# DongSky/few-shot-vit

Hardware: AMD Instinct MI355X
Metric: episodes_per_sec_5way_5shot_visformer_s (higher is better)
Workload: dtype bf16; 1 GPU; BASELINE configs[1]: Visformer-S (visformer_micro_80) miniImageNet-shaped 5-way 5-shot episodic eval, 15 query/class, 80x80 fp32 NCHW episodes resident in HBM, procedural weights + calibrated BN; images_per_episode=100, encoder_chunk_images=12800, distinct_episode_batches=16, parallelism=episode-parallel x1, one all-reduce of accuracy stats, ranks_seen=1, per_rank_eps=4521.1

## Files before the change

### few-shot-vit_amd/_lib.py

```python
import ctypes as C
import os

_HERE = os.path.dirname(os.path.abspath(__file__))
LIB_PATH = os.path.join(_HERE, 'libfsvit.so')

F32, BF16, F16, BF16X2, F16X2 = 0, 1, 2, 3, 4
ACT_NONE, ACT_GELU, ACT_LRELU = 0, 1, 2
HEAD_COS, HEAD_SQR, HEAD_DOT = 0, 1, 2
ERR_ARG, ERR_KEY, ERR_IMG_SIZE, ERR_WORKSPACE = -1, -2, -3, -4


class Tensor(C.Structure):
    _fields_ = [('name', C.c_char_p), ('data', C.POINTER(C.c_float)), ('ndim', C.c_int),
                ('shape', C.c_int64 * 4)]


class VisformerCfg(C.Structure):
    _fields_ = [('img_size', C.c_int), ('init_channels', C.c_int), ('embed_dim', C.c_int),
                ('depth', C.c_int * 3), ('num_heads', C.c_int), ('mlp_ratio', C.c_float),
                ('group', C.c_int), ('bn_eps', C.c_float)]


class VitCfg(C.Structure):
    _fields_ = [('img_size', C.c_int), ('patch_size', C.c_int), ('embed_dim', C.c_int), ('depth', C.c_int),
# ... 57 lines not shown
    'fsvit_soft_target_ce': (_i, [_fp, _fp, _fp, _fp, _i, _i, _f, _vp]),
    'fsvit_row_normalize': (_i, [_fp, _fp, _fp, _i, _i, _vp]),
    'fsvit_row_normalize_backward': (_i, [_fp, _fp, _fp, _fp, _i, _i, _vp]),
    'fsvit_adamw_step': (_i, [_fp, _fp, _fp, _fp, _sz, _f, _f, _f, _f, _f, _i, _vp]),
    'fsvit_adamw_step_multi': (_i, [_vp, _i, _sz, _f, _f, _f, _f, _f, _i, _vp]),
    'fsvit_proj_mlp_rows': (_i, [_vp, _vp, _vp, _vp, _i, _i, _vp, _i, _fp, _vp, _i, _fp, _i, _i, _i, _vp]),
    'fsvit_ln_linear_rows': (_i, [_vp, _vp, _vp, _i, _fp, _i, _i, _i, _f, _vp]),
    'fsvit_patch_embed2x2': (_i, [_vp, _vp, _vp, _i, _fp, _fp, _i, _i, _i, _i, _vp]),
    'fsvit_vit_block_tail': (_i, [_vp, _vp, _vp, _vp, _i, _i, _fp, _vp, _i, _fp, _vp, _i, _fp, _i, _i, _i, _f, _vp]),
    'fsvit_mlp_rows': (_i, [_vp, _vp, _vp, _i, _fp, _vp, _i, _fp, _i, _i, _i, _vp]),
    'fsvit_attention': (_i, [_vp, _vp, _i, _i, _i, _i, _f, _i, _vp]),
    'fsvit_qkv_attention': (_i, [_vp, _vp, _i, _fp, _vp, _i, _i, _i, _i, _i, _f, _vp]),
    'fsvit_vit_ln_qkv_attention': (_i, [_vp, _vp, _i, _fp, _vp, _i, _i, _i, _i, _i, _f, _f, _vp]),
    'fsvit_im2col27': (_i, [_fp, _vp, _i, _i, _i, _i, _vp]),
    'fsvit_stem_conv1': (_i, [_fp, _vp, _i, _fp, _vp, _vp, _i, _i, _i, _vp]),
    'fsvit_maxpool2_pos': (_i, [_vp, _fp, _vp, _i, _i, _i, _i, _i, _vp]),
    'fsvit_pool_affine': (_i, [_vp, _fp, _fp, _fp, _i, _i, _i, _i, _vp]),
    'fsvit_visformer_trainer_create': (_i, [C.POINTER(VisformerCfg), _i, C.POINTER(_vp)]),
    'fsvit_visformer_trainer_destroy': (None, [_vp]),
    'fsvit_visformer_trainer_workspace_bytes': (_sz, [_vp, C.POINTER(Param), _i, _i, _f]),
    'fsvit_visformer_train_forward': (_i, [_vp, C.POINTER(Param), _i, _fp, _i, _i, _i, _f, _fp, _fp, _vp, _sz, _vp]),
    'fsvit_visformer_train_backward': (_i, [_vp, C.POINTER(Param), _i, _fp, _vp]),
    'fsvit_vit_trainer_create': (_i, [C.POINTER(VitCfg), _i, C.POINTER(_vp)]),
    'fsvit_vit_trainer_destroy': (None, [_vp]),
    'fsvit_vit_trainer_droppath_calls': (_i, [_vp, _f]),
    'fsvit_vit_trainer_workspace_bytes': (_sz, [_vp, C.POINTER(Param), _i, _i, _f]),
    'fsvit_vit_train_forward': (_i, [_vp, C.POINTER(Param), _i, _fp, _i, _i, _i, _f, _fp, _fp, _vp, _sz, _vp]),
    'fsvit_vit_train_backward': (_i, [_vp, C.POINTER(Param), _i, _fp, _vp]),
    'fsvit_proto_head_backward': (_i, [_fp, _fp, _fp, _i, _i, _i, _i, _i, _f, _fp, _fp, _fp, _vp]),
    'fsvit_proto_head_backward_sqr': (_i, [_fp, _fp, _fp, _i, _i, _i, _i, _i, _f, _fp, _fp, _fp, _vp]),
# ... 82 lines not shown
```

### few-shot-vit_amd/csrc/conv3x3_halo.hip

```cpp
#include <stdlib.h>

#include <type_traits>
#include <utility>

#include "conv_gemm.h"
#include "fsvit_common.h"

namespace FSVIT_NS {

__device__ __attribute__((aligned(256))) unsigned char g_zero_page_halo[256];
typedef __attribute__((address_space(3))) void* lptrh_t;

__device__ __forceinline__ void hdma1(const void* gsrc, unsigned lds_byte_addr) {
  unsigned keep;
  asm volatile(
      "s_mov_b32 %0, m0\n\t"
      "s_mov_b32 m0, %2\n\t"
      "s_nop 0\n\t"
      "global_load_lds_dwordx4 %1, off\n\t"
      "s_mov_b32 m0, %0"
      : "=&s"(keep)
      : "v"(gsrc), "s"(lds_byte_addr)
      : "memory");
}
// ... 35 lines not shown
constexpr int NPIECE = 7;
constexpr int HBUF = 8 * PLANE;
constexpr int NST = 3, STAGE = 16384;
constexpr int OFF_W = 2 * HBUF;
constexpr int LDS_BYTES = OFF_W + NST * STAGE;
static_assert(LDS_BYTES == 160 * 1024, "the two halo buffers and the weight ring fill the LDS exactly");
}

template <int... I, typename F>
__device__ __forceinline__ void static_for_impl(std::integer_sequence<int, I...>, F&& f) {
  (f(std::integral_constant<int, I>{}), ...);
}
template <int N, typename F>
__device__ __forceinline__ void static_for(F&& f) { static_for_impl(std::make_integer_sequence<int, N>{}, static_cast<F&&>(f)); }

template <int CIN, bool FUSE_TAIL, bool STATS = false, int CREAL = CIN>
__global__ __launch_bounds__(512, 2) void conv3x3_halo_kernel(const ConvGemmParams p, const int n_tiles) {
  using namespace halo;
  extern __shared__ __attribute__((aligned(16))) unsigned char smem[];
  constexpr int NH = CIN / 64;
  constexpr int NKM = 9 * NH, NKT = NKM + (FUSE_TAIL ? 1 : 0);
  constexpr int MT = 5, NT = 4;
  const int t = threadIdx.x, lane = t & 63;
  const int wave = __builtin_amdgcn_readfirstlane(t >> 6);
  const int wm = wave >> 1, wn = wave & 1;
  const int lrow = lane & 15, lq = lane >> 4;
  const unsigned lds0 = (unsigned)(size_t)(lptrh_t)smem;
  unsigned char* const wst0 = smem + OFF_W;

  const unsigned char* const Xb = reinterpret_cast<const unsigned char*>(p.x);
  const unsigned char* const Wb = reinterpret_cast<const unsigned char*>(p.w);
  bf16* __restrict__ Y = reinterpret_cast<bf16*>(p.y);
  const int tiles_per_img = p.H / TR;
// ... 27 lines not shown
  auto issue_piece = [&](int j, int lane_o, const unsigned char* base, bool top, bool bot, int nb) {
    const int s = j * 64 + lane_o, hr = s / HP, hc = s - hr * HP;
    const bool ok = (base != nullptr) & (s < HR * HP) & (hc >= 1) & (hc <= TW) & !(top & (hr == 0)) & !(bot & (hr == HR - 1));
    const unsigned long a = (unsigned long)base + (unsigned long)(unsigned)(hr * x_rs + (hc - 1) * x_ps);
    const unsigned long z = (unsigned long)g_zero_page_halo;
    hdma1(reinterpret_cast<const void*>(ok ? a : z), lds0 + nb * HBUF + wave * PLANE + j * 1024);
  };
  auto halo_base = [&](int tile, int h) {
    const int bb = tile / tiles_per_img, rr = (tile - bb * tiles_per_img) * TR;
    if constexpr (CREAL != CIN) {
      if (h * 64 + wave * 8 >= CREAL) return (const unsigned char*)nullptr;
    }
    return Xb + (long)(bb * p.H + rr - 1) * x_rs + (p.x_planar ? (h * 8 + wave) * p.W * 16 : h * 128 + wave * 16);
  };

  f32x4 acc[MT][NT];
#pragma unroll
  for (int i = 0; i < MT; ++i)
#pragma unroll
    for (int j = 0; j < NT; ++j) acc[i][j] = f32x4{0.f, 0.f, 0.f, 0.f};

  int tix = blockIdx.x;
  if (tix >= n_tiles) return;
  const int my_tiles = (n_tiles - tix + (int)gridDim.x - 1) / (int)gridDim.x;
  int steps_left = my_tiles * NKT;

  auto wk_of = [&](int q) { return q >= NKM ? NKM : (NH == 2 ? (q >= 9 ? (q - 9) * 2 + 1 : q * 2) : q); };

  {
    const int r00 = (tix % tiles_per_img) * TR;
    const unsigned char* b0 = halo_base(tix, 0);
#pragma unroll
    for (int j = 0; j < NPIECE; ++j) issue_piece(j, lane, b0, r00 == 0, r00 + TR == p.H, 0);
  }
  issue_w(wk_of(0), 0);
  issue_w(wk_of(1 % NKT), 1);
  HWAIT(0);
  hbar();
  int st_cur = 0, st_pre = 2, q_pre = 2 % NKT;
  int buf = 0;
#define H_STAMP(acc_)

  auto advance = [&]() {
    st_cur = st_cur == NST - 1 ? 0 : st_cur + 1;
    st_pre = st_pre == NST - 1 ? 0 : st_pre + 1;
    q_pre = q_pre == NKT - 1 ? 0 : q_pre + 1;
    --steps_left;
  };

  while (true) {
    const int tnext = tix + (int)gridDim.x;
    const bool has_next = tnext < n_tiles;
    const int b = tix / tiles_per_img, r0 = (tix - b * tiles_per_img) * TR;
// ... 30 lines not shown
#pragma unroll
          for (int i = 0; i < MT; ++i) xf1[i] = *reinterpret_cast<const u32x4*>(smem + xb[i] + 4 * PLANE + TOFF);
        }
#pragma unroll
        for (int i = 0; i < MT; ++i)
#pragma unroll
          for (int j = 0; j < NT; ++j) acc[i][j] = mma_chunk<bf16>(wf0[j], xf0[i], acc[i][j]);
#pragma unroll
        for (int k = 0; k < MT + NT; ++k) {
          __builtin_amdgcn_sched_group_barrier(0x008, 1, 0);
          __builtin_amdgcn_sched_group_barrier(0x100, 1, 0);
        }
        __builtin_amdgcn_sched_group_barrier(0x008, MT * NT - (MT + NT), 0);
        __builtin_amdgcn_sched_barrier(0);
        H_STAMP(ckA);
        if (TAP >= 1 && TAP <= NPIECE) { if (pre_w) HWAIT(3); else HWAIT(1); }
        else { if (pre_w) HWAIT(2); else HWAIT(0); }
        H_STAMP(ckV);
        hbar();
        H_STAMP(ckW);
        if constexpr (TAP < NPIECE) issue_piece(TAP, lane_o, nbase, n_top, n_bot, buf ^ 1);
        const int st_next = st_cur == NST - 1 ? 0 : st_cur + 1;
        if constexpr (TAP < 8) {
          const unsigned char* wb = wst0 + st_next * STAGE + b_rd;
#pragma unroll
          for (int j = 0; j < NT; ++j) wf0[j] = *reinterpret_cast<const u32x4*>(wb + j * 2048 + sw0);
#pragma unroll
          for (int i = 0; i < MT; ++i) xf0[i] = *reinterpret_cast<const u32x4*>(smem + xb[i] + TOFF_N);
        } else if (FUSE_TAIL) {
          if (h == NH - 1) {
            const bf16* X2 = reinterpret_cast<const bf16*>(p.x2);
#pragma unroll
            for (int i = 0; i < MT; ++i) {
              const int lr = lane_o & 15;
              const int fr_o = ((lr >> 3) & 1) * 2 + ((lr >> 1) & 1), fc_o = ((lr >> 2) & 1) * 2 + (lr & 1);
              const size_t pix = (size_t)(b * p.H + r0 + blk_r(i) * 4 + fr_o) * p.W + blk_c(i) * 4 + fc_o;
              xf0[i] = hgload16(X2 + pix * p.x2_cstride + lq * 8);
            }
          }
        }
#pragma unroll
        for (int i = 0; i < MT; ++i)
#pragma unroll
          for (int j = 0; j < NT; ++j) acc[i][j] = mma_chunk<bf16>(wf1[j], xf1[i], acc[i][j]);
        if constexpr (TAP < NPIECE) {
#pragma unroll
          for (int k = 0; k < 8; ++k) {
            __builtin_amdgcn_sched_group_barrier(0x008, 1, 0);
            __builtin_amdgcn_sched_group_barrier(0x002, 3, 0);
          }
#pragma unroll
          for (int k = 0; k < MT + NT; ++k) {
            __builtin_amdgcn_sched_group_barrier(0x008, 1, 0);
            __builtin_amdgcn_sched_group_barrier(0x100, 1, 0);
          }
          __builtin_amdgcn_sched_group_barrier(0x008, MT * NT - 8 - (MT + NT), 0);
        } else if constexpr (TAP < 8) {
#pragma unroll
          for (int k = 0; k < MT + NT; ++k) {
            __builtin_amdgcn_sched_group_barrier(0x008, 1, 0);
// ... 185 lines not shown
  if (p.Cin != p.x_cstride || p.K != 9 * p.Cin) return false;
  if (p.stats && (p.pool2 || p.act != ACT_NONE)) return false;
  if (p.y_planar && (p.pool2 || p.stats)) return false;
  if (p.pool2) return p.Cin == 128 && p.x2 && p.K2 == 32 && p.x2_cstride >= 32 && p.pos && p.Kw == p.K + 64;
  return (p.Cin == 64 || p.Cin == 128) && !p.x2 && !p.pos && p.Kw == p.K;
}

static inline int halo_grid(const ConvGemmParams& p) { const int n_tiles = p.B * (p.H / halo::TR); return n_tiles < 256 ? n_tiles : 256; }
int conv3x3_halo_stats_rows(const ConvGemmParams& p, int dtype) {
  ConvGemmParams q = p;
  float dummy;
  q.stats = &dummy;
  return conv3x3_halo_eligible(q, dtype) ? halo_grid(p) : 0;
}

template <int CIN, bool FUSE_TAIL, bool STATS = false, int CREAL = CIN>
static int launch_halo_t(const ConvGemmParams& p, hipStream_t stream) {
  const int n_tiles = p.B * (p.H / halo::TR);
  auto kern = conv3x3_halo_kernel<CIN, FUSE_TAIL, STATS, CREAL>;
  hipError_t e = hipFuncSetAttribute((const void*)kern, hipFuncAttributeMaxDynamicSharedMemorySize, halo::LDS_BYTES);
  if (e != hipSuccess) return (int)e;
  const int grid = n_tiles < 256 ? n_tiles : 256;
  hipLaunchKernelGGL(kern, dim3(grid), dim3(512), halo::LDS_BYTES, stream, p, n_tiles);
  return (int)hipGetLastError();
}

int launch_conv3x3_halo(const ConvGemmParams& p, hipStream_t stream) {
  if (p.w_cpad) return p.pool2 ? launch_halo_t<128, true, false, 96>(p, stream) : launch_halo_t<128, false, false, 96>(p, stream);
  if (p.pool2) return launch_halo_t<128, true>(p, stream);
  if (p.stats) return p.Cin == 64 ? launch_halo_t<64, false, true>(p, stream) : launch_halo_t<128, false, true>(p, stream);
  return p.Cin == 64 ? launch_halo_t<64, false>(p, stream) : launch_halo_t<128, false>(p, stream);
}

}
```

### few-shot-vit_amd/csrc/conv_gemm.h

```cpp
#pragma once
#include <stddef.h>
#include <hip/hip_runtime.h>

namespace fsvit_types {


enum Act { ACT_NONE = 0, ACT_GELU = 1, ACT_LRELU = 2, ACT_MUL = 3 };

struct ConvGemmParams {
  const void* x;
  const void* w;
  const float* bias;
  const void* res;
  const float* pos;
  void* y;
  int B, H, W;
  int Cin;
  int x_cstride;
  int OH, OW;
  int KH, KW, stride, pad;
  int N;
  int y_cstride;
  int K;
  int Kw;
// ... 3 lines not shown
  int res_first;
  int log2Cin;
  const void* x2;
  int x2_cstride;
  int K2;
  int pool2;
  int y_rpi, y_row0;
  long w_gstride, w_rstride;
  int out_f32;
  void* y2;
  float* stats;
  int x_planar = 0, y_planar = 0;
  int w_cpad = 0;
};

}

#define FSVIT_DECLARE_CONV_GEMM(NS)                                                                                        \
  namespace NS {                                                                                                           \
  using namespace fsvit_types;                                                                                             \
  int launch_conv_gemm(const ConvGemmParams& p, int dtype, hipStream_t stream);                                            \
  int conv_gemm_route(const ConvGemmParams& p, int dtype);  \
  int launch_conv_gemm_v2(const ConvGemmParams& p, int dtype, hipStream_t stream);                                         \
   \
  bool gemm256_eligible(const ConvGemmParams& p, int dtype);                                                               \
  int launch_gemm256(const ConvGemmParams& p, hipStream_t stream);                                                         \
  int launch_gemm256_x2(const ConvGemmParams& p, hipStream_t stream);      \
        \
  bool conv3x3_halo_eligible(const ConvGemmParams& p, int dtype);                                                          \
  int launch_conv3x3_halo(const ConvGemmParams& p, hipStream_t stream);                                                    \
  int conv_stats_rows(const ConvGemmParams& p, int dtype);  \
  int conv3x3_halo_stats_rows(const ConvGemmParams& p, int dtype);                                                           \
  int conv_gemm_v2_config(const ConvGemmParams& p);                \
       \
  bool gconv3x3_x2_eligible(const ConvGemmParams& p, int dtype);                                                           \
  int launch_gconv3x3_x2(const ConvGemmParams& p, hipStream_t stream);                                                     \
  }
FSVIT_DECLARE_CONV_GEMM(fsvit)
FSVIT_DECLARE_CONV_GEMM(fsvit_f16)
```

### few-shot-vit_amd/csrc/engine.hip

```cpp
#include "../../include/fsvit.h"

#include <hip/hip_runtime.h>

#include <cmath>
#include <cstdarg>
#include <cstdio>
#include <cstring>
#include <cstdlib>
#include <utility>
#include <cstdint>
#include <initializer_list>
#include <map>
#include <string>
#include <vector>

#include "kernels.h"
#include "train_kernels.h"

using namespace fsvit;

#define K(fn) ((kdt == FSVIT_F16 || kdt == FSVIT_F16X2) ? fsvit_f16::fn : fsvit::fn)
static inline bool is_x2(int dtype) { return dtype == FSVIT_BF16X2 || dtype == FSVIT_F16X2; }
static inline bool known_dtype(int dtype) { return dtype >= FSVIT_F32 && dtype <= FSVIT_F16X2; }
static inline int kd(int dtype) { return (dtype == FSVIT_F32 || is_x2(dtype)) ? 0 : 1; }
// ... 553 lines not shown
    RC_TRY(upload(h, t, false, &d)); h->fshift = (float*)d;
  }
  return 0;
}

struct Plan {
  size_t patches, c1, c2;
  size_t ha, hb;
  size_t qkv, ctx, hid;
  size_t x1, x1b, x2, x3;
  size_t total;
};

size_t align256(size_t v) { return (v + 255) / 256 * 256; }

Plan make_plan(const fsvit_visformer* h, size_t Bc) {
  Plan p;
  const size_t es = h->es, P0 = (size_t)h->H0 * h->H0, P1 = (size_t)h->H1 * h->H1, P2 = (size_t)h->H2 * h->H2, P3 = (size_t)h->H3 * h->H3;
  const int heads = h->cfg.num_heads;
  size_t off = 0;
  auto take = [&](size_t bytes) { size_t o = off; off += align256(bytes); return o; };
  p.x1 = take(Bc * P1 * h->C1 * es);
  p.x1b = take(Bc * P1 * h->C1 * es);
  p.x2 = take(Bc * P2 * h->C2 * es);
  p.x3 = take(Bc * P3 * h->C3 * es);
  const size_t scratch0 = off;
  p.patches = take(Bc * P0 * 32 * es);
  p.c1 = take(Bc * P0 * h->C0 * es);
  p.c2 = take(Bc * P0 * h->C1 * es);
  size_t hi = off;
  off = scratch0;
  p.ha = take(Bc * P1 * h->hid1 * es);
  p.hb = take(Bc * P1 * h->hid1 * es);
  if (off > hi) hi = off;
  off = scratch0;
  size_t q2 = Bc * P2 * 3 * heads * h->hdp2 * es, q3 = Bc * P3 * 3 * heads * h->hdp3 * es;
  size_t c2 = Bc * P2 * heads * h->hdp2 * es, c3 = Bc * P3 * heads * h->hdp3 * es;
  size_t h2 = Bc * P2 * h->hid2 * es, h3 = Bc * P3 * h->hid3 * es;
  p.qkv = take(q2 > q3 ? q2 : q3);
  p.ctx = take(c2 > c3 ? c2 : c3);
  p.hid = take(h2 > h3 ? h2 : h3);
  if (off > hi) hi = off;
  p.total = hi;
  return p;
// ... 28 lines not shown

template <typename F>
int timed(EngineBase* h, hipStream_t st, const char* layer, int kernel, double flops, F&& launch) {
  if (!h->profiling) return launch();
  hipEvent_t e0 = h->prof_last, e1;
  if (!e0) { HIP_TRY(hipEventCreate(&e0)); HIP_TRY(hipEventRecord(e0, st)); }
  int rc = launch();
  if (rc != 0) return rc;
  HIP_TRY(hipEventCreate(&e1));
  HIP_TRY(hipEventRecord(e1, st));
  h->prof.push_back(ProfEntry{layer, kernel, flops, e0, e1});
  h->prof_last = e1;
  return 0;
}

static constexpr int stem_slice_images() { return 3200; }

int run_gemm(EngineBase* h, hipStream_t st, const char* layer, const Layer& L, const ConvGemmParams& p, double n_true, double k_true) {
  const int kdt = h->dtype;
  const double flops = 2.0 * (double)p.M * n_true * k_true * (double)p.groups;
  static const int kid_of_cfg[4] = {KID_GEMM256, KID_GEMM64, KID_GEMM32, KID_GEMM128};
  const int route = K(conv_gemm_route)(p, kg(kdt));
  const int kid = route == 0 ? KID_HALO : route == 1 ? KID_GEMM256 : route == 3 ? KID_GCONV_X2 : kid_of_cfg[K(conv_gemm_v2_config)(p)];
  return timed(h, st, layer, kid, flops, [&]() { return K(launch_conv_gemm)(p, kg(kdt), st); });
}

int forward_chunk(fsvit_visformer* h, const float* x, int Bc, float* feat, unsigned char* ws, bool first, hipStream_t st,
                  const float* xsrc2 = nullptr, int B1 = 0) {
  const Plan pl = make_plan(h, Bc);
  const int kdt = h->dtype, dt = kd(kdt);
  const size_t es = h->es;
  const int heads = h->cfg.num_heads;
  void *patches = ws + pl.patches, *c1 = ws + pl.c1, *c2 = ws + pl.c2;
  void *x1 = ws + pl.x1, *x1b = ws + pl.x1b, *x2 = ws + pl.x2, *x3 = ws + pl.x3, *ha = ws + pl.ha, *hb = ws + pl.hb;
  void *qkv = ws + pl.qkv, *ctx = ws + pl.ctx, *hid = ws + pl.hid;
  const int img = h->cfg.img_size;

  h->prof_last = nullptr;
  if (!xsrc2) B1 = Bc;
  const bool conv1_fused = K(stem_conv1_supported)(dt, img, h->C0);
  ConvGemmParams p2 = conv_params(h->conv2, c1, c2, Bc, h->H0, h->H0, h->C0, h->C0, 3, 3, 1, 1, h->C1, ACT_LRELU, nullptr, 0, nullptr);
  ConvGemmParams p3 = conv_params(h->conv3f, c2, x1, Bc, h->H0, h->H0, h->C1, h->C1, 3, 3, 1, 1, h->C1, ACT_LRELU, nullptr, 0, h->pos1);
  p3.x2 = patches; p3.x2_cstride = 32; p3.K2 = 32; p3.pool2 = 1;
  const bool planar = conv1_fused && K(conv_gemm_route)(p2, kg(kdt)) == 0 && K(conv_gemm_route)(p3, kg(kdt)) == 0;
  p2.x_planar = p2.y_planar = p3.x_planar = planar ? 1 : 0;
  if (planar) {
    const int S = stem_slice_images();
    const size_t s_pat = (size_t)h->H0 * h->H0 * 32 * es, s_c1 = (size_t)h->H0 * h->H0 * h->C0 * es, s_c2 = (size_t)h->H0 * h->H0 * h->C1 * es,
                 s_x1 = (size_t)h->H1 * h->H1 * h->C1 * es;
    const double fl1 = 2.0 * 27.0 * h->C0 * h->H0 * h->H0;
    for (int g0 = 0; g0 < Bc; g0 += S) {
      const int g1 = g0 + S < Bc ? g0 + S : Bc;
      for (int part = 0; part < 2; ++part) {
        const int a = part == 0 ? g0 : (g0 > B1 ? g0 : B1), b = part == 0 ? (g1 < B1 ? g1 : B1) : g1;
        if (a >= b) continue;
        const float* src = part == 0 ? x + (size_t)a * 3 * img * img : xsrc2 + (size_t)(a - B1) * 3 * img * img;
        RC_TRY(timed(h, st, "stem.im2col+conv1", KID_STEMCONV1, fl1 * (b - a), [&]() {
          return K(launch_stem_conv1)(src, (unsigned char*)patches + a * s_pat, (unsigned char*)c1 + a * s_c1, h->conv1.w, h->conv1.Kw, h->conv1.bias, b - a, st, 1); }));
      }
      ConvGemmParams q2 = p2, q3 = p3;
      q2.x = (const unsigned char*)c1 + g0 * s_c1; q2.y = (unsigned char*)c2 + g0 * s_c2; q2.B = g1 - g0; q2.M = (g1 - g0) * q2.OH * q2.OW;
      q3.x = (const unsigned char*)c2 + g0 * s_c2; q3.x2 = (const unsigned char*)patches + g0 * s_pat; q3.y = (unsigned char*)x1 + g0 * s_x1;
      q3.B = g1 - g0; q3.M = (g1 - g0) * q3.OH * q3.OW;
      RC_TRY(run_gemm(h, st, "stem.conv2", h->conv2, q2, h->C1, 9.0 * h->C0));
      RC_TRY(run_gemm(h, st, "stem.conv3+down+pool", h->conv3f, q3, h->C1, 9.0 * h->C1 + 27.0));
    }
  } else {
    if (conv1_fused) {
      const double fl1 = 2.0 * 27.0 * h->C0 * h->H0 * h->H0;
      RC_TRY(timed(h, st, "stem.im2col+conv1", KID_STEMCONV1, fl1 * B1, [&]() {
        return K(launch_stem_conv1)(x, patches, c1, h->conv1.w, h->conv1.Kw, h->conv1.bias, B1, st, 0); }));
      if (Bc > B1)
        RC_TRY(timed(h, st, "stem.im2col+conv1", KID_STEMCONV1, fl1 * (Bc - B1), [&]() {
          return K(launch_stem_conv1)(xsrc2, (unsigned char*)patches + (size_t)B1 * h->H0 * h->H0 * 32 * es, (unsigned char*)c1 + (size_t)B1 * h->H0 * h->H0 * h->C0 * es,
                                   h->conv1.w, h->conv1.Kw, h->conv1.bias, Bc - B1, st, 0); }));
    } else {
      RC_TRY(timed(h, st, "stem.im2col", KID_IM2COL, 0.0, [&]() { return K(launch_im2col27)(x, patches, B1, img, img, h->H0, h->H0, dt, st); }));
      if (Bc > B1)
        RC_TRY(timed(h, st, "stem.im2col", KID_IM2COL, 0.0, [&]() {
// ... 516 lines not shown
  const int kdt = dtype;
  if (!known_dtype(dtype)) return fail(FSVIT_ERR_ARG, "unknown dtype %d", dtype);
  if (!x || !out || (H & 1) || (W & 1)) return fail(FSVIT_ERR_ARG, "bad argument");
  RC_TRY(K(launch_im2col27)(x, out, B, H, W, H / 2, W / 2, kd(dtype), (hipStream_t)stream));
  return 0;
}

extern "C" int fsvit_stem_conv1(const float* x, const void* w, int kw, const float* bias, void* patches, void* c1, int B, int H, int W, void* stream) {
  const int kdt = FSVIT_BF16;
  if (!x || !w || !patches || !c1 || kw < 32) return fail(FSVIT_ERR_ARG, "bad argument");
  if (H != W || !K(stem_conv1_supported)(1, H, 64)) return fail(FSVIT_ERR_ARG, "fsvit_stem_conv1: only 80x80 images, 64 output channels (bf16) are built");
  RC_TRY(K(launch_stem_conv1)(x, patches, c1, w, kw, bias, B, (hipStream_t)stream, 0));
  return 0;
}

extern "C" int fsvit_maxpool2_pos(const void* in, const float* pos, void* out, int B, int OH, int OW, int C, int dtype, void* stream) {
  const int kdt = dtype;
  if (!known_dtype(dtype)) return fail(FSVIT_ERR_ARG, "unknown dtype %d", dtype);
  if (!in || !out || C % 4) return fail(FSVIT_ERR_ARG, "bad argument");
  RC_TRY(K(launch_maxpool2_pos)(in, pos, out, B, OH, OW, C, kd(dtype), (hipStream_t)stream));
  return 0;
}

extern "C" int fsvit_pool_affine(const void* x, const float* scale, const float* shift, float* feat, int B, int HW, int C,
                                 int dtype, void* stream) {
  const int kdt = dtype;
  if (!known_dtype(dtype)) return fail(FSVIT_ERR_ARG, "unknown dtype %d", dtype);
  if (!x || !scale || !shift || !feat || C % 4) return fail(FSVIT_ERR_ARG, "bad argument");
  RC_TRY(K(launch_pool_affine)(x, scale, shift, feat, B, HW, C, kd(dtype), (hipStream_t)stream));
  return 0;
// ... 449 lines not shown
```

### few-shot-vit_amd/engine.py

```python
import ctypes as C
import os
import sys
from typing import Dict, Optional

import numpy as np
import torch

from . import _lib

DTYPES = {'f32': _lib.F32, 'parity': _lib.F32, 'fp32': _lib.F32, 'bf16': _lib.BF16, 'f16': _lib.F16, 'fp16': _lib.F16,
          'bf16x2': _lib.BF16X2, 'f16x2': _lib.F16X2}
TORCH_DTYPE = {_lib.F32: torch.float32, _lib.BF16: torch.bfloat16, _lib.F16: torch.float16, _lib.BF16X2: torch.float32, _lib.F16X2: torch.float32}
EVAL_ONLY = (_lib.F16, _lib.F16X2)


_tensor_generation = {}


def bump_weight_generation(tensors) -> None:
    for t in tensors:
        if t is not None:
            p = t.data_ptr()
            _tensor_generation[p] = _tensor_generation.get(p, 0) + 1

# ... 623 lines not shown
            _lib.check(lib.fsvit_im2col27(_ptr(x.contiguous()), _ptr(out), B, H, W, ops._dt(out), _stream_ptr(x.device)))
        return out

    @staticmethod
    def stem_conv1(x, w, bias):
        _require_cuda(x, w)
        lib = _lib.load()
        B, _, H, W = x.shape
        patches = torch.empty(B * (H // 2) * (W // 2), 32, dtype=w.dtype, device=x.device)
        c1 = torch.empty(B * (H // 2) * (W // 2), 64, dtype=w.dtype, device=x.device)
        with torch.cuda.device(x.device):
            _lib.check(lib.fsvit_stem_conv1(_ptr(x.contiguous()), _ptr(w), w.shape[-1], _ptr(bias), _ptr(patches), _ptr(c1), B, H, W, _stream_ptr(x.device)))
        return patches, c1

    @staticmethod
    def maxpool2_pos(x, pos):
        _require_cuda(x)
        lib = _lib.load()
        B, H, W, Cc = x.shape
        out = torch.empty(B, H // 2, W // 2, Cc, dtype=x.dtype, device=x.device)
        with torch.cuda.device(x.device):
            _lib.check(lib.fsvit_maxpool2_pos(_ptr(x), _ptr(pos), _ptr(out), B, H // 2, W // 2, Cc, ops._dt(x), _stream_ptr(x.device)))
        return out

    @staticmethod
    def pool_affine(x, scale, shift):
        _require_cuda(x)
        lib = _lib.load()
        B, HW, Cc = x.shape
        out = torch.empty(B, Cc, dtype=torch.float32, device=x.device)
# ... 395 lines not shown
```

### include/fsvit.h

```cpp
#ifndef FSVIT_H
#define FSVIT_H
#include <stddef.h>
#include <stdint.h>

#ifdef __cplusplus
extern "C" {
#endif

enum { FSVIT_F32 = 0, FSVIT_BF16 = 1, FSVIT_F16 = 2, FSVIT_BF16X2 = 3, FSVIT_F16X2 = 4 };
enum { FSVIT_ACT_NONE = 0, FSVIT_ACT_GELU = 1, FSVIT_ACT_LRELU = 2 };
enum { FSVIT_HEAD_COS = 0, FSVIT_HEAD_SQR = 1, FSVIT_HEAD_DOT = 2 };
enum {
  FSVIT_ERR_ARG = -1,
  FSVIT_ERR_KEY = -2,
  FSVIT_ERR_IMG_SIZE = -3,
  FSVIT_ERR_WORKSPACE = -4
};

const char* fsvit_last_error(void);
const char* fsvit_version(void);

typedef struct fsvit_visformer fsvit_visformer;

typedef struct fsvit_tensor {
// ... 116 lines not shown
int fsvit_linear_backward(const float* dy_dev, const float* x_dev, const float* w_dev, float* dx_dev, int accumulate_dx, float* dw_dev,
                          float* db_dev, int M, int N, int K, void* stream);
int fsvit_token_softlabel(const float* teacher_logits_dev, float* soft_dev, int B, int T, int C, int k, int bp, double smoothing, void* stream);
int fsvit_soft_target_ce(const float* logits_dev, const float* target_dev, float* row_loss_dev, float* dlogits_dev, int R, int C,
                         float grad_scale, void* stream);
int fsvit_row_normalize(const float* x_dev, float* y_dev, float* inv_norm_dev, int R, int D, void* stream);
int fsvit_row_normalize_backward(const float* y_dev, const float* inv_norm_dev, const float* dy_dev, float* dx_dev, int R, int D, void* stream);
int fsvit_adamw_step(float* p_dev, const float* g_dev, float* m_dev, float* v_dev, size_t n, float lr, float beta1, float beta2, float eps,
                     float weight_decay, int step, void* stream);
int fsvit_adamw_step_multi(const void* items_dev, int n_items, size_t max_numel, float lr, float beta1, float beta2, float eps, float weight_decay, int step,
                           void* stream);

int fsvit_im2col27(const float* x_nchw_dev, void* out_dev, int B, int H, int W, int dtype, void* stream);
int fsvit_stem_conv1(const float* x_nchw_dev, const void* w_dev, int kw, const float* bias_dev, void* patches_dev, void* c1_dev,
                     int B, int H, int W, void* stream);
int fsvit_maxpool2_pos(const void* in_dev, const float* pos_dev, void* out_dev, int B, int OH, int OW, int C,
                       int dtype, void* stream);
int fsvit_pool_affine(const void* x_dev, const float* scale_dev, const float* shift_dev, float* feat_dev,
                      int B, int HW, int C, int dtype, void* stream);

typedef struct fsvit_param {
  const char* name;
  float* data;
  float* grad;
  int64_t numel;
} fsvit_param;
typedef struct fsvit_visformer_trainer fsvit_visformer_trainer;
int fsvit_visformer_train_tokens(fsvit_visformer_trainer* t, float* tokens_dev, void* stream);
int fsvit_visformer_train_set_token_grad(fsvit_visformer_trainer* t, const float* dtokens_dev);
int fsvit_visformer_trainer_create(const fsvit_visformer_cfg* cfg, int dtype, fsvit_visformer_trainer** out);
// ... 105 lines not shown
```

Before: 4518 episodes/s.

## Fuse stem im2col and conv1 into the halo conv2 kernel

The stem's im2col+conv1 stage is folded into the 3x3 halo conv2 kernel. Each tile's fp32 input window is DMA'd into LDS, gathered into 27-tap patches, run through a bf16 MMA with LeakyReLU, and written directly into the halo buffer as conv2's input. The c1 activation no longer makes a round trip through HBM, a separate kernel launch per slice goes away, and the scratch buffers shrink to slice size. In exchange the kernel recomputes conv1 on halo rows, interleaves the new work into the conv2 tap pipeline, and adds register pressure.

```diff
diff --git a/few-shot-vit_amd/_lib.py b/few-shot-vit_amd/_lib.py
--- a/few-shot-vit_amd/_lib.py
+++ b/few-shot-vit_amd/_lib.py
@@ -95,6 +95,7 @@
     'fsvit_vit_ln_qkv_attention': (_i, [_vp, _vp, _i, _fp, _vp, _i, _i, _i, _i, _i, _f, _f, _vp]),
     'fsvit_im2col27': (_i, [_fp, _vp, _i, _i, _i, _i, _vp]),
     'fsvit_stem_conv1': (_i, [_fp, _vp, _i, _fp, _vp, _vp, _i, _i, _i, _vp]),
+    'fsvit_stem_conv12': (_i, [_fp, _vp, _i, _fp, _vp, _i, _fp, _vp, _vp, _i, _i, _i, _i, _vp]),
     'fsvit_maxpool2_pos': (_i, [_vp, _fp, _vp, _i, _i, _i, _i, _i, _vp]),
     'fsvit_pool_affine': (_i, [_vp, _fp, _fp, _fp, _i, _i, _i, _i, _vp]),
     'fsvit_visformer_trainer_create': (_i, [C.POINTER(VisformerCfg), _i, C.POINTER(_vp)]),
diff --git a/few-shot-vit_amd/csrc/conv3x3_halo.hip b/few-shot-vit_amd/csrc/conv3x3_halo.hip
--- a/few-shot-vit_amd/csrc/conv3x3_halo.hip
+++ b/few-shot-vit_amd/csrc/conv3x3_halo.hip
@@ -73,9 +73,10 @@
 template <int N, typename F>
 __device__ __forceinline__ void static_for(F&& f) { static_for_impl(std::make_integer_sequence<int, N>{}, static_cast<F&&>(f)); }
 
-template <int CIN, bool FUSE_TAIL, bool STATS = false, int CREAL = CIN>
-__global__ __launch_bounds__(512, 2) void conv3x3_halo_kernel(const ConvGemmParams p, const int n_tiles) {
+template <int CIN, bool FUSE_TAIL, bool STATS = false, int CREAL = CIN, bool FUSE_C1 = false>
+__global__ __launch_bounds__(512, 2) void conv3x3_halo_kernel(const ConvGemmParams p, const int n_tiles, const HaloConv1Params f1) {
   using namespace halo;
+  static_assert(!FUSE_C1 || (CIN == 64 && !FUSE_TAIL && !STATS && CREAL == CIN), "conv1 is fused into the 64-channel plain variant only");
   extern __shared__ __attribute__((aligned(16))) unsigned char smem[];
   constexpr int NH = CIN / 64;
   constexpr int NKM = 9 * NH, NKT = NKM + (FUSE_TAIL ? 1 : 0);
@@ -133,6 +134,99 @@
     return Xb + (long)(bb * p.H + rr - 1) * x_rs + (p.x_planar ? (h * 8 + wave) * p.W * 16 : h * 128 + wave * 16);
   };
 
+  constexpr int C1_IR = 2 * HR + 1, C1_IW = 80, C1_PIX = HR * TW, C1_MT = (C1_PIX + 15) / 16, C1_PER = (C1_MT + 7) / 8;
+  constexpr int C1_NP = 3;
+  static_assert(!FUSE_C1 || (C1_NP * 8 * 1024 >= 3 * C1_IR * C1_IW * 4 && C1_NP * 8 * 1024 <= HBUF), "the fp32 window fits the pieces, the pieces fit the buffer");
+  auto c1_image = [&](int tile) {
+    const int bb = tile / tiles_per_img;
+    return bb < f1.B1 ? f1.x0 + (size_t)bb * 3 * C1_IW * C1_IW : f1.x1 + (size_t)(bb - f1.B1) * 3 * C1_IW * C1_IW;
+  };
+  auto c1_piece = [&](int j, int lane_o, int tile, int nb) {
+    const int pid = j * 8 + wave, fi = pid * 64 + lane_o;
+    const int c = fi / (C1_IR * (C1_IW / 4)), rem = fi - c * (C1_IR * (C1_IW / 4)), r = rem / (C1_IW / 4), q4 = rem - r * (C1_IW / 4);
+    const int iy = tile >= 0 ? 2 * ((tile % tiles_per_img) * TR) - 3 + r : -1;
+    const bool ok = (tile >= 0) & (fi < 3 * C1_IR * (C1_IW / 4)) & (iy >= 0) & (iy < C1_IW);
+    const float* img = c1_image(tile >= 0 ? tile : 0);
+    const unsigned long a = (unsigned long)(img + ((c * C1_IW + iy) * C1_IW + q4 * 4));
+    const unsigned long z = (unsigned long)g_zero_page_halo;
+    hdma1(reinterpret_cast<const void*>(ok ? a : z), lds0 + nb * HBUF + pid * 1024);
+  };
+  u32x4 c1w[FUSE_C1 ? 4 : 1];
+  f32x4 c1b[FUSE_C1 ? 4 : 1];
+  if constexpr (FUSE_C1) {
+    const bf16* w1 = reinterpret_cast<const bf16*>(f1.w1);
+#pragma unroll
+    for (int ct = 0; ct < 4; ++ct) {
+      const int pp = ct >> 1, hh = ct & 1;
+      c1w[ct] = *reinterpret_cast<const u32x4*>(w1 + (size_t)(32 * pp + 8 * (lrow >> 2) + 4 * hh + (lrow & 3)) * f1.kw1 + 8 * lq);
+      c1b[ct] = f1.b1 ? *reinterpret_cast<const f32x4*>(f1.b1 + 32 * pp + 8 * lq + 4 * hh) : f32x4{0.f, 0.f, 0.f, 0.f};
+    }
+  }
+  u32x4 c1q[FUSE_C1 ? C1_PER : 1];
+  auto c1_gather = [&](int lane_o, int tile, int nb) {
+    const int m_o = lane_o & 15, lq_o = lane_o >> 4;
+    const float* win = reinterpret_cast<const float*>(smem + nb * HBUF);
+    const int bb = tile / tiles_per_img, r0t = (tile - bb * tiles_per_img) * TR;
+    constexpr int KNONE = -(1 << 20);
+    int koff[8];
+    bool kx0[8];
+#pragma unroll
+    for (int j = 0; j < 8; ++j) {
+      const int k = 8 * lq_o + j, tp = k / 3, c = k - 3 * tp, ky = tp / 3, kx = tp - 3 * ky;
+      koff[j] = k < 27 ? (c * C1_IR + ky) * C1_IW + kx - 1 : KNONE;
+      kx0[j] = kx == 0;
+    }
+    bf16* pat = reinterpret_cast<bf16*>(f1.patches);
+#pragma unroll
+    for (int i = 0; i < C1_PER; ++i) {
+      const int tl = wave + 8 * i;
+      if (tl < C1_MT) {
+        const int px = tl * 16 + m_o, hr = px / TW, ox = px - hr * TW;
+        const int org = 2 * hr * C1_IW + 2 * ox;
+        unsigned short e[8];
+#pragma unroll
+        for (int j = 0; j < 8; ++j) {
+          const bool okj = (koff[j] != KNONE) & !(kx0[j] & (ox == 0));
+          const float v = win[okj ? org + koff[j] : 0];
+          e[j] = okj ? __builtin_bit_cast(unsigned short, (bf16)v) : (unsigned short)0;
+        }
+        const u32x4 pf = {(unsigned)e[0] | ((unsigned)e[1] << 16), (unsigned)e[2] | ((unsigned)e[3] << 16), (unsigned)e[4] | ((unsigned)e[5] << 16),
+                          (unsigned)e[6] | ((unsigned)e[7] << 16)};
+        c1q[i] = pf;
+        if (hr >= 1 && hr <= TR)
+          *reinterpret_cast<u32x4*>(pat + ((size_t)(bb * p.H + r0t + hr - 1) * TW + ox) * 32 + 8 * lq_o) = pf;
+      }
+    }
+  };
+  auto c1_mma = [&](int i, int lane_o, int tile, int nb) {
+    const int tl = wave + 8 * i;
+    if (tl >= C1_MT) return;
+    const int m_o = lane_o & 15, lq_o = lane_o >> 4;
+    const int r0t = (tile % tiles_per_img) * TR;
+    const int px = tl * 16 + m_o, hr = px / TW, ox = px - hr * TW;
+    const int y = r0t - 1 + hr;
+    const bool inside = (y >= 0) & (y < p.H);
+    unsigned char* dst = smem + nb * HBUF + lq_o * PLANE + (hr * HP + ox + 1) * 16;
+#pragma unroll
+    for (int pp = 0; pp < 2; ++pp) {
+      const f32x4 a0 = mma_chunk<bf16>(c1w[2 * pp], c1q[i], c1b[2 * pp]), a1 = mma_chunk<bf16>(c1w[2 * pp + 1], c1q[i], c1b[2 * pp + 1]);
+      bf16x8 o;
+#pragma unroll
+      for (int q = 0; q < 4; ++q) {
+        o[q] = (bf16)fmaxf(a0[q], 0.1f * a0[q]);
+        o[4 + q] = (bf16)fmaxf(a1[q], 0.1f * a1[q]);
+      }
+      const u32x4 ov = __builtin_bit_cast(u32x4, o);
+      *reinterpret_cast<u32x4*>(dst + pp * 4 * PLANE) = inside ? ov : u32x4{0u, 0u, 0u, 0u};
+    }
+  };
+  auto c1_border = [&](int t_o, int nb) {
+    if (t_o < 8 * HR * 2) {
+      const int pl = t_o / (HR * 2), rem = t_o - pl * (HR * 2), hr = rem >> 1, hc = (rem & 1) ? TW + 1 : 0;
+      *reinterpret_cast<u32x4*>(smem + nb * HBUF + pl * PLANE + (hr * HP + hc) * 16) = u32x4{0u, 0u, 0u, 0u};
+    }
+  };
+
   f32x4 acc[MT][NT];
 #pragma unroll
   for (int i = 0; i < MT; ++i)
@@ -146,7 +240,10 @@
 
   auto wk_of = [&](int q) { return q >= NKM ? NKM : (NH == 2 ? (q >= 9 ? (q - 9) * 2 + 1 : q * 2) : q); };
 
-  {
+  if constexpr (FUSE_C1) {
+#pragma unroll
+    for (int j = 0; j < C1_NP; ++j) c1_piece(j, lane, tix, 0);
+  } else {
     const int r00 = (tix % tiles_per_img) * TR;
     const unsigned char* b0 = halo_base(tix, 0);
 #pragma unroll
@@ -156,6 +253,17 @@
   issue_w(wk_of(1 % NKT), 1);
   HWAIT(0);
   hbar();
+  if constexpr (FUSE_C1) {
+    c1_gather(lane, tix, 0);
+    HWAIT(0);
+    hbar();
+#pragma unroll
+    for (int i = 0; i < C1_PER; ++i) c1_mma(i, lane, tix, 0);
+    c1_border(t, 0);
+    HWAIT(0);
+    hbar();
+  }
+  constexpr int NPC = FUSE_C1 ? C1_NP : NPIECE;
   int st_cur = 0, st_pre = 2, q_pre = 2 % NKT;
   int buf = 0;
 #define H_STAMP(acc_)
@@ -216,12 +324,22 @@
         __builtin_amdgcn_sched_group_barrier(0x008, MT * NT - (MT + NT), 0);
         __builtin_amdgcn_sched_barrier(0);
         H_STAMP(ckA);
-        if (TAP >= 1 && TAP <= NPIECE) { if (pre_w) HWAIT(3); else HWAIT(1); }
+        if (TAP >= 1 && TAP <= NPC) { if (pre_w) HWAIT(3); else HWAIT(1); }
         else { if (pre_w) HWAIT(2); else HWAIT(0); }
         H_STAMP(ckV);
         hbar();
         H_STAMP(ckW);
-        if constexpr (TAP < NPIECE) issue_piece(TAP, lane_o, nbase, n_top, n_bot, buf ^ 1);
+        if constexpr (FUSE_C1) {
+          if constexpr (TAP < C1_NP) c1_piece(TAP, lane_o, n_tix, buf ^ 1);
+          else if constexpr (TAP == 4) { if (has_next) c1_gather(lane_o, n_tix, buf ^ 1); }
+          else if constexpr (TAP == 5) {
+            if (has_next) {
+              c1_mma(0, lane_o, n_tix, buf ^ 1);
+              c1_mma(1, lane_o, n_tix, buf ^ 1);
+              c1_border(lane_o + wave * 64, buf ^ 1);
+            }
+          } else if constexpr (TAP == 6 || TAP == 7) { if (has_next) c1_mma(TAP - 4, lane_o, n_tix, buf ^ 1); }
+        } else if constexpr (TAP < NPIECE) issue_piece(TAP, lane_o, nbase, n_top, n_bot, buf ^ 1);
         const int st_next = st_cur == NST - 1 ? 0 : st_cur + 1;
         if constexpr (TAP < 8) {
           const unsigned char* wb = wst0 + st_next * STAGE + b_rd;
@@ -245,7 +363,7 @@
         for (int i = 0; i < MT; ++i)
 #pragma unroll
           for (int j = 0; j < NT; ++j) acc[i][j] = mma_chunk<bf16>(wf1[j], xf1[i], acc[i][j]);
-        if constexpr (TAP < NPIECE) {
+        if constexpr (TAP < NPC) {
 #pragma unroll
           for (int k = 0; k < 8; ++k) {
             __builtin_amdgcn_sched_group_barrier(0x008, 1, 0);
@@ -461,14 +579,14 @@
   return conv3x3_halo_eligible(q, dtype) ? halo_grid(p) : 0;
 }
 
-template <int CIN, bool FUSE_TAIL, bool STATS = false, int CREAL = CIN>
-static int launch_halo_t(const ConvGemmParams& p, hipStream_t stream) {
+template <int CIN, bool FUSE_TAIL, bool STATS = false, int CREAL = CIN, bool FUSE_C1 = false>
+static int launch_halo_t(const ConvGemmParams& p, hipStream_t stream, const HaloConv1Params& f1 = HaloConv1Params{}) {
   const int n_tiles = p.B * (p.H / halo::TR);
-  auto kern = conv3x3_halo_kernel<CIN, FUSE_TAIL, STATS, CREAL>;
+  auto kern = conv3x3_halo_kernel<CIN, FUSE_TAIL, STATS, CREAL, FUSE_C1>;
   hipError_t e = hipFuncSetAttribute((const void*)kern, hipFuncAttributeMaxDynamicSharedMemorySize, halo::LDS_BYTES);
   if (e != hipSuccess) return (int)e;
   const int grid = n_tiles < 256 ? n_tiles : 256;
-  hipLaunchKernelGGL(kern, dim3(grid), dim3(512), halo::LDS_BYTES, stream, p, n_tiles);
+  hipLaunchKernelGGL(kern, dim3(grid), dim3(512), halo::LDS_BYTES, stream, p, n_tiles, f1);
   return (int)hipGetLastError();
 }
 
@@ -479,4 +597,13 @@
   return p.Cin == 64 ? launch_halo_t<64, false>(p, stream) : launch_halo_t<128, false>(p, stream);
 }
 
-}
+bool conv3x3_halo_c1_eligible(const ConvGemmParams& p, int dtype) {
+  return conv3x3_halo_eligible(p, dtype) && p.Cin == 64 && !p.stats && !p.pool2 && !p.w_cpad && p.H == 40 && p.act != ACT_GELU;
+}
+
+int launch_conv3x3_halo_c1(const ConvGemmParams& p, const HaloConv1Params& f1, hipStream_t stream) {
+  if (p.B <= 0) return 0;
+  return launch_halo_t<64, false, false, 64, true>(p, stream, f1);
+}
+
+}
diff --git a/few-shot-vit_amd/csrc/conv_gemm.h b/few-shot-vit_amd/csrc/conv_gemm.h
--- a/few-shot-vit_amd/csrc/conv_gemm.h
+++ b/few-shot-vit_amd/csrc/conv_gemm.h
@@ -41,6 +41,16 @@
   int w_cpad = 0;
 };
 
+struct HaloConv1Params {
+  const float* x0 = nullptr;
+  const float* x1 = nullptr;
+  int B1 = 0;
+  const void* w1 = nullptr;
+  int kw1 = 0;
+  const float* b1 = nullptr;
+  void* patches = nullptr;
+};
+
 }
 
 #define FSVIT_DECLARE_CONV_GEMM(NS)                                                                                        \
@@ -56,6 +66,8 @@
         \
   bool conv3x3_halo_eligible(const ConvGemmParams& p, int dtype);                                                          \
   int launch_conv3x3_halo(const ConvGemmParams& p, hipStream_t stream);                                                    \
+  bool conv3x3_halo_c1_eligible(const ConvGemmParams& p, int dtype);                                                       \
+  int launch_conv3x3_halo_c1(const ConvGemmParams& p, const HaloConv1Params& f1, hipStream_t stream);                      \
   int conv_stats_rows(const ConvGemmParams& p, int dtype);  \
   int conv3x3_halo_stats_rows(const ConvGemmParams& p, int dtype);                                                           \
   int conv_gemm_v2_config(const ConvGemmParams& p);                \
diff --git a/few-shot-vit_amd/csrc/engine.hip b/few-shot-vit_amd/csrc/engine.hip
--- a/few-shot-vit_amd/csrc/engine.hip
+++ b/few-shot-vit_amd/csrc/engine.hip
@@ -591,6 +591,9 @@
 
 size_t align256(size_t v) { return (v + 255) / 256 * 256; }
 
+bool stem_fused_route(const fsvit_visformer* h);
+constexpr int stem_slice_images();
+
 Plan make_plan(const fsvit_visformer* h, size_t Bc) {
   Plan p;
   const size_t es = h->es, P0 = (size_t)h->H0 * h->H0, P1 = (size_t)h->H1 * h->H1, P2 = (size_t)h->H2 * h->H2, P3 = (size_t)h->H3 * h->H3;
@@ -602,9 +605,16 @@
   p.x2 = take(Bc * P2 * h->C2 * es);
   p.x3 = take(Bc * P3 * h->C3 * es);
   const size_t scratch0 = off;
-  p.patches = take(Bc * P0 * 32 * es);
-  p.c1 = take(Bc * P0 * h->C0 * es);
-  p.c2 = take(Bc * P0 * h->C1 * es);
+  if (stem_fused_route(h)) {
+    const size_t Ss = Bc < (size_t)stem_slice_images() ? Bc : (size_t)stem_slice_images();
+    p.patches = take(Ss * P0 * 32 * es);
+    p.c1 = p.patches;
+    p.c2 = take(Ss * P0 * h->C1 * es);
+  } else {
+    p.patches = take(Bc * P0 * 32 * es);
+    p.c1 = take(Bc * P0 * h->C0 * es);
+    p.c2 = take(Bc * P0 * h->C1 * es);
+  }
   size_t hi = off;
   off = scratch0;
   p.ha = take(Bc * P1 * h->hid1 * es);
@@ -663,7 +673,16 @@
   return 0;
 }
 
-static constexpr int stem_slice_images() { return 3200; }
+constexpr int stem_slice_images() { return 3200; }
+
+bool stem_fused_route(const fsvit_visformer* h) {
+  const int kdt = h->dtype;
+  if (!K(stem_conv1_supported)(kd(kdt), h->cfg.img_size, h->C0)) return false;
+  ConvGemmParams p2 = conv_params(h->conv2, nullptr, nullptr, 1, h->H0, h->H0, h->C0, h->C0, 3, 3, 1, 1, h->C1, ACT_LRELU, nullptr, 0, nullptr);
+  ConvGemmParams p3 = conv_params(h->conv3f, nullptr, nullptr, 1, h->H0, h->H0, h->C1, h->C1, 3, 3, 1, 1, h->C1, ACT_LRELU, nullptr, 0, h->pos1);
+  p3.x2_cstride = 32; p3.K2 = 32; p3.pool2 = 1; p3.x2 = h->pos1;
+  return K(conv_gemm_route)(p2, kg(kdt)) == 0 && K(conv_gemm_route)(p3, kg(kdt)) == 0 && K(conv3x3_halo_c1_eligible)(p2, kg(kdt));
+}
 
 int run_gemm(EngineBase* h, hipStream_t st, const char* layer, const Layer& L, const ConvGemmParams& p, double n_true, double k_true) {
   const int kdt = h->dtype;
@@ -691,27 +710,25 @@
   ConvGemmParams p2 = conv_params(h->conv2, c1, c2, Bc, h->H0, h->H0, h->C0, h->C0, 3, 3, 1, 1, h->C1, ACT_LRELU, nullptr, 0, nullptr);
   ConvGemmParams p3 = conv_params(h->conv3f, c2, x1, Bc, h->H0, h->H0, h->C1, h->C1, 3, 3, 1, 1, h->C1, ACT_LRELU, nullptr, 0, h->pos1);
   p3.x2 = patches; p3.x2_cstride = 32; p3.K2 = 32; p3.pool2 = 1;
-  const bool planar = conv1_fused && K(conv_gemm_route)(p2, kg(kdt)) == 0 && K(conv_gemm_route)(p3, kg(kdt)) == 0;
+  const bool planar = stem_fused_route(h);
   p2.x_planar = p2.y_planar = p3.x_planar = planar ? 1 : 0;
   if (planar) {
     const int S = stem_slice_images();
-    const size_t s_pat = (size_t)h->H0 * h->H0 * 32 * es, s_c1 = (size_t)h->H0 * h->H0 * h->C0 * es, s_c2 = (size_t)h->H0 * h->H0 * h->C1 * es,
-                 s_x1 = (size_t)h->H1 * h->H1 * h->C1 * es;
+    const size_t s_x1 = (size_t)h->H1 * h->H1 * h->C1 * es, s_img = (size_t)3 * img * img;
     const double fl1 = 2.0 * 27.0 * h->C0 * h->H0 * h->H0;
     for (int g0 = 0; g0 < Bc; g0 += S) {
-      const int g1 = g0 + S < Bc ? g0 + S : Bc;
-      for (int part = 0; part < 2; ++part) {
-        const int a = part == 0 ? g0 : (g0 > B1 ? g0 : B1), b = part == 0 ? (g1 < B1 ? g1 : B1) : g1;
-        if (a >= b) continue;
-        const float* src = part == 0 ? x + (size_t)a * 3 * img * img : xsrc2 + (size_t)(a - B1) * 3 * img * img;
-        RC_TRY(timed(h, st, "stem.im2col+conv1", KID_STEMCONV1, fl1 * (b - a), [&]() {
-          return K(launch_stem_conv1)(src, (unsigned char*)patches + a * s_pat, (unsigned char*)c1 + a * s_c1, h->conv1.w, h->conv1.Kw, h->conv1.bias, b - a, st, 1); }));
-      }
+      const int g1 = g0 + S < Bc ? g0 + S : Bc, n = g1 - g0;
+      HaloConv1Params f1;
+      f1.B1 = B1 <= g0 ? 0 : (B1 >= g1 ? n : B1 - g0);
+      f1.x0 = x + (size_t)g0 * s_img;
+      f1.x1 = xsrc2 ? xsrc2 + (size_t)((g0 > B1 ? g0 : B1) - B1) * s_img : nullptr;
+      f1.w1 = h->conv1.w; f1.kw1 = h->conv1.Kw; f1.b1 = h->conv1.bias; f1.patches = patches;
       ConvGemmParams q2 = p2, q3 = p3;
-      q2.x = (const unsigned char*)c1 + g0 * s_c1; q2.y = (unsigned char*)c2 + g0 * s_c2; q2.B = g1 - g0; q2.M = (g1 - g0) * q2.OH * q2.OW;
-      q3.x = (const unsigned char*)c2 + g0 * s_c2; q3.x2 = (const unsigned char*)patches + g0 * s_pat; q3.y = (unsigned char*)x1 + g0 * s_x1;
-      q3.B = g1 - g0; q3.M = (g1 - g0) * q3.OH * q3.OW;
-      RC_TRY(run_gemm(h, st, "stem.conv2", h->conv2, q2, h->C1, 9.0 * h->C0));
+      q2.x = nullptr; q2.y = c2; q2.B = n; q2.M = n * q2.OH * q2.OW;
+      q3.x = c2; q3.x2 = patches; q3.y = (unsigned char*)x1 + g0 * s_x1;
+      q3.B = n; q3.M = n * q3.OH * q3.OW;
+      RC_TRY(timed(h, st, "stem.conv2+im2col+conv1", KID_HALO, fl1 * n + 2.0 * (double)q2.M * h->C1 * 9.0 * h->C0, [&]() {
+        return K(launch_conv3x3_halo_c1)(q2, f1, st); }));
       RC_TRY(run_gemm(h, st, "stem.conv3+down+pool", h->conv3f, q3, h->C1, 9.0 * h->C1 + 27.0));
     }
   } else {
@@ -1258,6 +1275,21 @@
   return 0;
 }
 
+extern "C" int fsvit_stem_conv12(const float* x, const void* w1, int kw1, const float* bias1, const void* w2, int kw2, const float* bias2, void* patches,
+                                 void* c2, int B, int H, int W, int c2_planar, void* stream) {
+  const int kdt = FSVIT_BF16;
+  if (!x || !w1 || !w2 || !patches || !c2 || kw1 < 32 || B < 0) return fail(FSVIT_ERR_ARG, "bad argument");
+  if (H != W || !K(stem_conv1_supported)(1, H, 64)) return fail(FSVIT_ERR_ARG, "fsvit_stem_conv12: only 80x80 images, 64 -> 128 channels (bf16) are built");
+  Layer L; L.w = const_cast<void*>(w2); L.bias = const_cast<float*>(bias2); L.N = 128; L.K = 9 * 64; L.Kw = kw2; L.groups = 1;
+  ConvGemmParams p = conv_params(L, nullptr, c2, B, H / 2, W / 2, 64, 64, 3, 3, 1, 1, 128, ACT_LRELU, nullptr, 0, nullptr);
+  p.x_planar = 1; p.y_planar = c2_planar ? 1 : 0;
+  if (!K(conv3x3_halo_c1_eligible)(p, 1)) return fail(FSVIT_ERR_ARG, "fsvit_stem_conv12: kw2 must be 576 (9 taps x 64 channels)");
+  HaloConv1Params f1;
+  f1.x0 = x; f1.B1 = B; f1.w1 = w1; f1.kw1 = kw1; f1.b1 = bias1; f1.patches = patches;
+  RC_TRY(K(launch_conv3x3_halo_c1)(p, f1, (hipStream_t)stream));
+  return 0;
+}
+
 extern "C" int fsvit_maxpool2_pos(const void* in, const float* pos, void* out, int B, int OH, int OW, int C, int dtype, void* stream) {
   const int kdt = dtype;
   if (!known_dtype(dtype)) return fail(FSVIT_ERR_ARG, "unknown dtype %d", dtype);
diff --git a/few-shot-vit_amd/engine.py b/few-shot-vit_amd/engine.py
--- a/few-shot-vit_amd/engine.py
+++ b/few-shot-vit_amd/engine.py
@@ -661,6 +661,18 @@
         return patches, c1
 
     @staticmethod
+    def stem_conv12(x, w1, bias1, w2, bias2, planar=False):
+        _require_cuda(x, w1, w2)
+        lib = _lib.load()
+        B, _, H, W = x.shape
+        patches = torch.empty(B * (H // 2) * (W // 2), 32, dtype=w1.dtype, device=x.device)
+        c2 = torch.empty((B, H // 2, 16, W // 2, 8) if planar else (B, H // 2, W // 2, 128), dtype=w1.dtype, device=x.device)
+        with torch.cuda.device(x.device):
+            _lib.check(lib.fsvit_stem_conv12(_ptr(x.contiguous()), _ptr(w1), w1.shape[-1], _ptr(bias1), _ptr(w2), w2.shape[-1], _ptr(bias2),
+                                             _ptr(patches), _ptr(c2), B, H, W, int(planar), _stream_ptr(x.device)))
+        return patches, c2
+
+    @staticmethod
     def maxpool2_pos(x, pos):
         _require_cuda(x)
         lib = _lib.load()
diff --git a/include/fsvit.h b/include/fsvit.h
--- a/include/fsvit.h
+++ b/include/fsvit.h
@@ -154,6 +154,8 @@
 int fsvit_im2col27(const float* x_nchw_dev, void* out_dev, int B, int H, int W, int dtype, void* stream);
 int fsvit_stem_conv1(const float* x_nchw_dev, const void* w_dev, int kw, const float* bias_dev, void* patches_dev, void* c1_dev,
                      int B, int H, int W, void* stream);
+int fsvit_stem_conv12(const float* x_nchw_dev, const void* w1_dev, int kw1, const float* bias1_dev, const void* w2_dev, int kw2, const float* bias2_dev,
+                      void* patches_dev, void* c2_dev, int B, int H, int W, int c2_planar, void* stream);
 int fsvit_maxpool2_pos(const void* in_dev, const float* pos_dev, void* out_dev, int B, int OH, int OW, int C,
                        int dtype, void* stream);
 int fsvit_pool_affine(const void* x_dev, const float* scale_dev, const float* shift_dev, float* feat_dev,
```

Measured after the change: 4562 episodes/s (median of 6 runs). No clear change (+1.0%).
